# ittiam-systems/libxaac

Hardware: AMD Instinct MI355X
Metric: decoded audio frames/s (1024-spl IMDCT + complex QMF + HQ SBR + parametric stereo, HE-AACv2) (higher is better)
Workload: dtype int32

## Files before the change

### libxaac_amd/csrc/sbr_core.h

```cpp
#ifndef XAAC_SBR_CORE_H
#define XAAC_SBR_CORE_H

#include "fx.h"
#include "../../include/xaac_sbr.h"

#ifndef XS_TABLES_DECLARED
#define XS_TABLES_DECLARED
#if defined(__HIPCC__)
#define XAAC_TAB_QUAL static __device__ const
#include "tables_sbr.inc"
#undef XAAC_TAB_QUAL
#else
#include "tables_sbr.inc"
#endif
#endif

#define XS_MAXF XAAC_SBR_MAX_FREQ_COEFFS

FX_HD int32_t xs_shl(int32_t v, int s) { return (int32_t)((uint32_t)v << (s & 31)); }
FX_HD int32_t xs_sar(int32_t v, int s) { return v >> (s & 31); }
FX_HD int xs_pnorm32(int32_t a) { return fx_norm32(a); }
FX_HD int16_t xs_mult16_shl_sat(int16_t a, int16_t b) { return fx_sat16(((int32_t)a * b) >> 15); }
FX_HD int16_t xs_mult16_shl(int16_t a, int16_t b) { return (int16_t)(((int32_t)a * b) >> 15); }
FX_HD int16_t xs_mult16(int16_t a, int16_t b) { return (int16_t)(((int32_t)a * b) >> 16); }
// ... 317 lines not shown
  return r;
}

template <int HQ_, int NB_ = 64, int LD_ = 0, int NS_ = 32>
struct XsQmfT {
  static constexpr int HQ = HQ_;
  static constexpr int NB = NB_;
  static constexpr int LD = LD_;
  static constexpr int NS = NS_;
  static constexpr int OV = LD_ ? 0 : 6;
  static constexpr int IM = NB_;
  static constexpr int ROW = HQ_ ? 2 * NB_ : NB_;
  int32_t *p;
  FX_MEMBER int32_t &operator()(int slot, int band) const { return p[(slot + 2) * ROW + band]; }
  FX_MEMBER int32_t &im(int slot, int band) const { return p[(slot + 2) * ROW + IM + band]; }
};
typedef XsQmfT<0> XsQmf;
typedef XsQmfT<1> XsQmfHq;

struct XsCov {
  int32_t phi_11, phi_22, phi_01, phi_02, phi_12, d;
};

struct XsWork {
  int32_t bw_array[XAAC_SBR_MAX_PATCHES];
  union {
    int32_t fold_a[XS_MAXF + 8][2];
    int16_t nrg_est[2 * XS_MAXF];
  };
  int32_t fold_b[XS_MAXF + 8][4];
// ... 2132 lines not shown
      a0r = (int16_t)(xs_shl(fx_mul32x16(fx_sub_sat(0, tr), inv), norm + 1) >> 15);
    if (fx_abs_sat(ti) >= p11)
      reset = 1;
    else
      a0i = (int16_t)(xs_shl(fx_mul32x16(fx_sub_sat(0, ti), inv), norm + 1) >> 15);
  }
  if (fx_add_sat((int32_t)a0r * a0r, (int32_t)a0i * a0i) >= 0x40000000) reset = 1;
  if (fx_add_sat((int32_t)a1r * a1r, (int32_t)a1i * a1i) >= 0x40000000) reset = 1;
  if (reset) a0r = a0i = a1r = a1i = 0;
  a[0] = a0r;
  a[1] = a0i;
  a[2] = a1r;
  a[3] = a1i;
}

template <class Q>
FX_HD void xs_patch_band_hq(const xaac_sbr_header *h, const Q &x, int lb, int hb, const int16_t *alpha,
                            const int32_t *bw_array, int start_idx, int stop_idx) {
  constexpr int kBwCap = XAAC_SBR_MAX_PATCHES - 1 < XAAC_SBR_MAX_NOISE_VALUES ? XAAC_SBR_MAX_PATCHES - 1 : XAAC_SBR_MAX_NOISE_VALUES;
  int bord[kBwCap];
  XS_UNROLL
  for (int i = 0; i < kBwCap; i++) bord[i] = h->bw_borders[i];
  int bi = 0;
  bool on = true;
  XS_UNROLL
  for (int i = 0; i < kBwCap; i++) {
    on = on && hb >= bord[i];
    bi += on ? 1 : 0;
  }
  int16_t bw = (int16_t)(bw_array[bi] >> 16);
  const int16_t a0r = xs_mult16_shl_sat(bw, alpha[0]), a0i = xs_mult16_shl_sat(bw, alpha[1]);
  bw = xs_mult16_shl_sat(bw, bw);
  const int16_t a1r = xs_mult16_shl_sat(bw, alpha[2]), a1i = xs_mult16_shl_sat(bw, alpha[3]);
  const int n = stop_idx - start_idx;
  const bool filt = bw > 0;
  const int16_t c0r = filt ? a0r : (int16_t)0, c0i = filt ? a0i : (int16_t)0, c1r = filt ? a1r : (int16_t)0,
                c1i = filt ? a1i : (int16_t)0;
  int32_t p2r = x(start_idx - 2, lb), p2i = x.im(start_idx - 2, lb);
  int32_t p1r = x(start_idx - 1, lb), p1i = x.im(start_idx - 1, lb);
  XS_UNROLL4
  for (int i = 0; i < n; i++) {
    const int32_t cr = x(start_idx + i, lb), ci = x.im(start_idx + i, lb);
    int32_t acc = fx_sub(fx_add(fx_sub(fx_mul32x16(p1r, c0r), fx_mul32x16(p1i, c0i)), fx_mul32x16(p2r, c1r)),
                         fx_mul32x16(p2i, c1i));
    x(start_idx + i, hb) = fx_add(cr >> 2, fx_shlw(acc, 1));
    acc = fx_add(fx_add_sat(fx_add_sat(fx_mul32x16(p1r, c0i), fx_mul32x16(p1i, c0r)), fx_mul32x16(p2r, c1i)),
                 fx_mul32x16(p2i, c1r));
    x.im(start_idx + i, hb) = fx_add(ci >> 2, fx_shlw(acc, 1));
    p2r = p1r;
    p2i = p1i;
    p1r = cr;
    p1i = ci;
  }
}

template <class ST, class Q>
FX_HD void xs_hf_generator_hq(const XsCx &cx, const xaac_sbr_header *h, ST *st, const Q &x, XsWork *w,
                              int start_idx, int last_slot_offset, int max_qmf_subband, const int32_t *invf_mode,
                              const int32_t *invf_mode_prev) {
  const int num_patches = cx.uni(h->num_patches);
  const int stop_idx = cx.uni(h->num_columns) + last_slot_offset;
  XS_PAR(i, 0, XAAC_SBR_MAX_PATCHES) w->bw_array[i] = 0;
  cx.sync();
  xs_invfilt_level_emphasis(cx, st->bw_array_prev, h->num_if_bands, invf_mode, invf_mode_prev, w->bw_array);
  const int actual_stop = cx.uni(
      (int16_t)(h->patch[num_patches - 1].dst_start_band + h->patch[num_patches - 1].num_bands_in_patch));
  {
    const int nz = actual_stop < Q::NB ? Q::NB - actual_stop : 0;
    XS_PAR(c, 0, 2 * nz) {
      const int col = c < nz ? actual_stop + c : Q::IM + actual_stop + (c - nz);
      XS_UNROLL4
      for (int l = start_idx; l < stop_idx; l++) x(l, col) = 0;
    }
  }
  const int start_patch = cx.uni(h->start_patch), stop_patch = cx.uni(h->stop_patch);
  XS_PAR(k, start_patch, stop_patch) {
    x(-2, k) = st->lpc_real[0][k];
    x(-1, k) = st->lpc_real[1][k];
    x.im(-2, k) = st->lpc_imag[0][k];
    x.im(-1, k) = st->lpc_imag[1][k];
  }
  cx.sync();
  XS_T(12);
  XsLv al01, al23, src;
  al01.fill(0);
  al23.fill(0);
  const int ncov = Q::LD ? cx.uni(h->num_columns) : Q::NS + 6;
// ... 50 lines not shown
  XS_LANES(hb, 0, 64) wide |= src.own(hb) >= 0 && (hb < max_qmf_subband || hb >= max_qmf_subband + 32);
  if (cx.wave_or(wide) == 0 && max_qmf_subband >= 0 && stop_idx - start_idx >= 8) {
    XsLv idx;
    idx.fill(0);
    XS_LANES(l, 0, 64) idx.own(l) = (max_qmf_subband + (l & 31)) & 63;
    const XsLv src2 = src.gather(idx);
    XsLv srcc;
    srcc.fill(0);
    XS_LANES(l, 0, 64) srcc.own(l) = (max_qmf_subband + (l & 31) < 64) ? src2.own(l) : -1;
    const XsLv b01 = al01.gather(srcc), b23 = al23.gather(srcc);
    const int mid = start_idx + ((stop_idx - start_idx + 1) >> 1);
    XS_LANES(l, 0, 64) {
      const int lb = srcc.own(l), hb = max_qmf_subband + (l & 31);
      if (lb >= 0) {
        const int16_t alpha[4] = {xs_m(b01.own(l)), xs_e(b01.own(l)), xs_m(b23.own(l)), xs_e(b23.own(l))};
        xs_patch_band_hq(h, x, lb, hb, alpha, w->bw_array, l < 32 ? start_idx : mid, l < 32 ? mid : stop_idx);
      }
    }
  } else {
    const XsLv a01 = al01.gather(src), a23 = al23.gather(src);
    XS_LANES(hb, 0, 64) {
      const int lb = src.own(hb);
      if (lb >= 0) {
        const int16_t alpha[4] = {xs_m(a01.own(hb)), xs_e(a01.own(hb)), xs_m(a23.own(hb)), xs_e(a23.own(hb))};
        xs_patch_band_hq(h, x, lb, hb, alpha, w->bw_array, start_idx, stop_idx);
      }
    }
  }
  cx.sync();
  XS_T(14);
  XS_PAR(i, 0, h->num_if_bands) st->bw_array_prev[i] = w->bw_array[i];
  cx.sync();
}

struct XsPendingAdjust {
  int b0, b1, first_start, sh_ov, sh_main;
};
template <class ST, class Q>
FX_HD int xs_calc_sbrenvelope(const XsCx &cx, const xaac_sbr_header *h, const xaac_sbr_frame *f,
                              const int16_t *env_sf_all, const int16_t *noise_floor_all, ST *st, const Q &x,
// ... 425 lines not shown
FX_HD int xs_sbr_core_tail(const XsCx &cx, const xaac_sbr_header *h, const xaac_sbr_frame *f, const int16_t *env_sf_all,
                           const int16_t *noise_floor_all, ST *st, const Q &x, XsWork *w, const int16_t *rand_hi,
                           const XsBfp &b, XsPendingAdjust *pend = nullptr, const int32_t *sf_words = nullptr) {
  const int save_lb_scale = b.save_lb_scale, max_samp_val = b.max_samp_val;
  (void)max_samp_val;
  if (cx.uni(f->apply_processing)) {
    XsLv deg64;
    deg64.fill(0);
    const int n_env = cx.uni(f->num_env), nts = cx.uni(h->num_time_slots), ts = cx.uni(h->time_step);
    const int16_t last = fx_sat16((int32_t)cx.uni(f->border_vec[n_env]) - nts);
    if constexpr (!Q::HQ)
      xs_low_pow_hf_generator(cx, h, st, x, w, deg64, cx.uni(f->border_vec[0]) * ts, ts * last,
                              cx.uni(f->max_qmf_subband_aac), f->sbr_invf_mode, st->prev_invf_mode, max_samp_val);
    else
      xs_hf_generator_hq(cx, h, st, x, w, cx.uni(f->border_vec[0]) * ts, ts * last, cx.uni(f->max_qmf_subband_aac),
                         f->sbr_invf_mode, st->prev_invf_mode);
    XS_T(2);
    XS_ONE st->hb_scale = (int16_t)((st->ov_lb_scale < st->lb_scale ? st->ov_lb_scale : st->lb_scale) - 2);
    cx.sync();
    if (xs_calc_sbrenvelope(cx, h, f, env_sf_all, noise_floor_all, st, x, w, rand_hi, deg64, pend, sf_words)) return -1;
    XS_PAR(i, 0, h->num_if_bands) st->prev_invf_mode[i] = f->sbr_invf_mode[i];
    XS_ONE {
      st->prev_coupling_mode = f->coupling_mode;
      st->prev_max_qmf_subband_aac = f->max_qmf_subband_aac;
      st->prev_end_position = f->border_vec[f->num_env];
      st->prev_amp_res = f->amp_res;
    }
  } else {
    XS_ONE st->hb_scale = (int16_t)save_lb_scale;
  }
  cx.sync();
// ... 30 lines not shown
```

### libxaac_amd/csrc/sbr_core_kernel.h

```cpp
#ifndef XAAC_SBR_CORE_KERNEL_H
#define XAAC_SBR_CORE_KERNEL_H

#include <hip/hip_runtime_api.h>
#include <stdint.h>

#include "../../include/xaac_amd.h"

#define XAAC_SBR_X_ROWS 40
#define XAAC_SBR_X_WORDS (XAAC_SBR_X_ROWS * 64)
#define XAAC_SBR_NARROW_BANDS 48
#ifndef XAAC_SBR_CORE_HQ_WAVES
#define XAAC_SBR_CORE_HQ_WAVES 4
#endif

typedef struct XaacSbrCoreParams {
  int32_t n_ch;
  const xaac_sbr_header *header;
  const xaac_sbr_frame *frame;
  xaac_sbr_state *state;
  int32_t *x;
  int16_t *syn_par;
  int32_t *status;
  int32_t *defer_list, *defer_count;
  int32_t *work_counter;
  int32_t num_cu;
  int32_t counters_zeroed;
  int32_t qmf_slots;
  int32_t narrow_only;
} XaacSbrCoreParams;

#ifdef __cplusplus
extern "C" {
#endif
hipError_t xaac_launch_sbr_core_lp(const XaacSbrCoreParams *p, hipStream_t stream);
hipError_t xaac_launch_sbr_screen(const XaacSbrCoreParams *p, hipStream_t stream);
hipError_t xaac_launch_sbr_core_hq(const XaacSbrCoreParams *p, hipStream_t stream);
#ifdef __cplusplus
}
#endif
#endif
```

### libxaac_amd/csrc/sbr_core_kernel.hip

```cpp
#include <hip/hip_runtime.h>
#include <stddef.h>
#include <stdint.h>
#include <stdlib.h>

#ifdef XS_PROFILE
__shared__ long long xs_prof_last[4];
__shared__ unsigned xs_prof_acc[4][32];
#define XS_T(i)                                                  \
  do {                                                           \
    if ((threadIdx.x & 63) == 0) {                               \
      long long t_ = clock64();                                  \
      xs_prof_acc[threadIdx.x >> 6][i] += (unsigned)(t_ - xs_prof_last[threadIdx.x >> 6]); \
      xs_prof_last[threadIdx.x >> 6] = t_;                       \
    }                                                            \
  } while (0)
#endif
__shared__ int16_t xs_lds_inv_table[256];
__shared__ int16_t xs_lds_sqrt_table[258];
__shared__ int32_t xs_lds_rand_ph[568];
__shared__ int16_t xs_lds_rand_hi[568];
__shared__ int16_t xs_lds_small16[8 + 4 + 50];
__shared__ int32_t xs_lds_new_bw[16];
#define XS_TAB_LIMG(i) xs_lds_small16[i]
#define XS_TAB_SMOOTH(i) xs_lds_small16[8 + (i)]
// ... 341 lines not shown
  for (int j = 0; j < NR; j++)
    if (tid + THREADS * j < 568) {
      if (HQ)
        xs_lds_rand_ph[tid + THREADS * j] = tr[j];
      else
        xs_lds_rand_hi[tid + THREADS * j] = (int16_t)(tr[j] >> 16);
    }
#pragma unroll
  for (int j = 0; j < NI; j++)
    if (tid + THREADS * j < 256) xs_lds_inv_table[tid + THREADS * j] = ti[j];
#pragma unroll
  for (int j = 0; j < NS; j++)
    if (tid + THREADS * j < 257) xs_lds_sqrt_table[tid + THREADS * j] = ts[j];
}

}

#ifndef XS_LP_MIN_WAVES
#define XS_LP_MIN_WAVES 3
#endif
template <int HQ, int NB, int WAVES, int NS = 32>
__global__ __launch_bounds__(64 * WAVES, HQ ? 1 : XS_LP_MIN_WAVES) void xaac_sbr_core_kernel(XaacSbrCoreParams p) {
  __shared__ XsLds<HQ, NB> s[WAVES];
  const int lane = threadIdx.x & 63, wave = __builtin_amdgcn_readfirstlane(threadIdx.x >> 6);
  stage_tables<HQ, 64 * WAVES>(threadIdx.x);
  __syncthreads();
  if (XS_STAGGER_G > 1 && p.work_counter && p.n_ch >= 3 * (int)gridDim.x * WAVES) {
    const int g = ((int)blockIdx.x * WAVES + wave) % XS_STAGGER_G;
    for (int t = 0; t < g; t++) __builtin_amdgcn_s_sleep(XS_STAGGER_SLEEP);
  }
// ... 18 lines not shown
}

template <int HQ, int NS = 32>
__global__ __launch_bounds__(64) void xaac_sbr_core_list_kernel(XaacSbrCoreParams p) {
  __shared__ XsLds<HQ, 64> s;
  const int lane = threadIdx.x;
  const int n = *p.defer_count;
  if ((int)blockIdx.x >= n) return;
  stage_tables<HQ, 64>(lane);
  for (int j = blockIdx.x; j < n; j += gridDim.x) {
    xs_wave_sync();
    core_one<HQ, 64, NS>(p, p.defer_list[j], s, lane);
  }
}

template <int NS>
static hipError_t launch_sbr_core_lp(const XaacSbrCoreParams *p, hipStream_t stream) {
  XaacSbrCoreParams q = *p;
  q.work_counter = nullptr;
#ifndef XS_LP_WAVES
#define XS_LP_WAVES 2
#endif
  constexpr int W = XS_LP_WAVES;
#ifndef XS_LP_PERSISTENT
#define XS_LP_PERSISTENT 1
#endif
  if (XS_LP_PERSISTENT && p->work_counter && p->counters_zeroed) {
#ifndef XS_LP_WG_PER_CU
#define XS_LP_WG_PER_CU 5
#endif
// ... 31 lines not shown
    q.work_counter = nullptr;
    hipLaunchKernelGGL((xaac_sbr_core_kernel<1, 64, 1, NS>), dim3(p->n_ch), dim3(64), 0, stream, q);
    return hipGetLastError();
  }
  if (!p->counters_zeroed) {
    hipError_t e = hipMemsetAsync(p->defer_count, 0, 2 * sizeof(int32_t), stream);
    if (e != hipSuccess) return e;
  }
  constexpr int W = XAAC_SBR_CORE_HQ_WAVES;
  static int per_cu = 0;
  if (!per_cu) {
    const char *e = getenv("XAAC_CORE_WG_PER_CU");
    per_cu = e && atoi(e) > 0 ? atoi(e) : 2;
  }
  const int resident = per_cu * (p->num_cu > 0 ? p->num_cu : 256), need = (p->n_ch + W - 1) / W;
  hipLaunchKernelGGL((xaac_sbr_core_kernel<1, XAAC_SBR_NARROW_BANDS, W, NS>), dim3(need < resident ? need : resident), dim3(64 * W), 0,
                     stream, *p);
  if (p->narrow_only) return hipGetLastError();
  const int grid = p->n_ch < 64 ? p->n_ch : 64;
  hipLaunchKernelGGL((xaac_sbr_core_list_kernel<1, NS>), dim3(grid), dim3(64), 0, stream, *p);
  return hipGetLastError();
}

extern "C" hipError_t xaac_launch_sbr_core_hq(const XaacSbrCoreParams *p, hipStream_t stream) {
  return p->qmf_slots == 30 ? launch_sbr_core_hq<30>(p, stream) : launch_sbr_core_hq<32>(p, stream);
}

extern "C" hipError_t xaac_warm_sbr_core(void) {
  hipFuncAttributes a;
  return hipFuncGetAttributes(&a, reinterpret_cast<const void *>(&xaac_sbr_core_kernel<1, XAAC_SBR_NARROW_BANDS, XAAC_SBR_CORE_HQ_WAVES, 32>));
}
```

### libxaac_amd/csrc/sbr_qmf_kernel.h

```cpp
#ifndef XAAC_SBR_QMF_KERNEL_H
#define XAAC_SBR_QMF_KERNEL_H

#include <hip/hip_runtime_api.h>
#include <stdint.h>

#include "../../include/xaac_amd.h"
#include "../../include/xaac_sbr.h"

#ifndef XAAC_QMF_WAVES
#define XAAC_QMF_WAVES 1
#endif
#define XAAC_QMF_BLOCK (64 * XAAC_QMF_WAVES)
#define XAAC_QMF_ANA_LDS_PER_WAVE (2 * 1312 * 2 + 32 + 64 * 65 * 4)
#define XAAC_QMF_SYN_LDS_PER_WAVE_LP 21376
#define XAAC_QMF_SYN_LDS_PER_WAVE_HQ (64 * 129 * 4)

typedef struct XaacQmfAnaParams {
  int32_t n_ch, ch_fac, low_pow, usb, slot_stride;
  int32_t state_stride;
  int32_t qmf_ch_stride;
  const int16_t *pcm;
  xaac_qmf_ana_state *state;
  int32_t *qmf;
  const xaac_sbr_frame *frame;
  int32_t *zero_words;
  int32_t n_slots;
  const int16_t *refused;
} XaacQmfAnaParams;

typedef struct XaacQmfSynParams {
  int32_t n_ch, ch_fac, low_pow, lsb, usb, split, slot_stride;
  int32_t state_stride, qmf_ch_stride;
  int32_t scale_stride;
  int32_t per_ch_bands;
  int32_t down_sample;
  const int32_t *qmf;
  const int16_t *scale;
  xaac_qmf_syn_state *state;
  int16_t *pcm;
  int32_t pcm_ch_stride, pcm_sample_stride;
// ... 43 lines not shown
```

### libxaac_amd/csrc/sbr_qmf_kernel.hip

```cpp
#include <hip/hip_runtime.h>
#include <stdint.h>

#include "sbr_qmf.h"
#include "sbr_qmf_kernel.h"

namespace {

constexpr int kHist = 288 + 1024;

__device__ __forceinline__ int ana_ring_pos(int wr, int a) {
  int p = wr + 32 + a;
  return p >= 320 ? p - 320 : p;
}

template <int NS = 32>
__device__ __forceinline__ int ana_phase_after_frame(int phase) {
  int f1 = phase, f2 = phase + 64;
  for (int s = 0; s < NS; s++) {
    f1 += 64;
    f2 += 64;
    int t = f1;
    f1 = f2;
    f2 = t;
    if (f2 > 640) {
// ... 13 lines not shown
}

template <bool LP, int NS = 32>
__global__ __launch_bounds__(XAAC_QMF_BLOCK) void xaac_qmf_analysis_kernel(XaacQmfAnaParams p) {
  extern __shared__ __attribute__((aligned(16))) char smem[];
  const int lane = threadIdx.x & 63;
  const int wave = __builtin_amdgcn_readfirstlane(threadIdx.x >> 6);
  char *wbase = smem + wave * XAAC_QMF_ANA_LDS_PER_WAVE;
  int16_t *hist = reinterpret_cast<int16_t *>(wbase);
  int32_t *z = reinterpret_cast<int32_t *>(wbase + 2 * kHist * 2 + 32);

  int32_t coef[5];
#pragma unroll
  for (int j = 0; j < 5; j++) coef[j] = xaac_qmf_qmf_c[2 * lane + 128 * j];

  if (p.zero_words && blockIdx.x == 0 && threadIdx.x < 2) p.zero_words[threadIdx.x] = 0;
  const int n_pairs = (p.n_ch + 1) >> 1;
  const int waves_total = gridDim.x * XAAC_QMF_WAVES;
  for (int pair = blockIdx.x * XAAC_QMF_WAVES + wave; pair < n_pairs; pair += waves_total) {
    int wr_v[2] = {0, 0}, ph_v[2] = {0, 0};
    {
      constexpr int NP = 32 * NS / 64;
      int16_t hr[2][5], hp[2][NP];
#pragma unroll
      for (int c = 0; c < 2; c++) {
        const int ch = 2 * pair + c;
        if (ch < p.n_ch) {
          const xaac_qmf_ana_state *st = reinterpret_cast<const xaac_qmf_ana_state *>(
              reinterpret_cast<const char *>(p.state) + (size_t)ch * p.state_stride);
          wr_v[c] = st->wr;
          ph_v[c] = st->phase;
// ... 102 lines not shown
        st->phase = (int16_t)ph_new;
      }
    }
  }
}

template <int NS = 32>
__global__ __launch_bounds__(128) void xaac_qmf_analysis_hq_kernel(XaacQmfAnaParams p) {
  __shared__ int16_t hist[2][kHist];
  __shared__ int32_t tile[2 * 64 * 33];
  const int lane = threadIdx.x & 63;
  const int w = __builtin_amdgcn_readfirstlane(threadIdx.x >> 6);
  const int pair = blockIdx.x;
  const int chw = 2 * pair + w;
  const bool live = chw < p.n_ch;
  if (p.zero_words && blockIdx.x == 0 && threadIdx.x < 2) p.zero_words[threadIdx.x] = 0;
  xaac_qmf_ana_state *st = reinterpret_cast<xaac_qmf_ana_state *>(reinterpret_cast<char *>(p.state) + (size_t)(live ? chw : 0) * p.state_stride);
  int wr = 0, phase_old = 0;
  int rot_apply = 0, rot_sub = 0, rot_usb = 0;
  const bool rot_live = p.frame && 2 * pair + (lane >> 5) < p.n_ch;
  if (rot_live) {
    const int ch = 2 * pair + (lane >> 5);
    const xaac_sbr_frame *f = p.frame + ch;
    const xaac_sbr_state *sst = reinterpret_cast<const xaac_sbr_state *>(reinterpret_cast<const char *>(p.state) + (size_t)ch * p.state_stride);
    rot_apply = f->apply_processing;
    rot_sub = f->max_qmf_subband_aac;
    rot_usb = sst->codec_usb;
  }
  {
    int16_t *h = hist[w];
    if (live) {
// ... 830 lines not shown
```

### libxaac_amd/csrc/xaac_abi.cpp

```cpp
#include <hip/hip_runtime_api.h>
#include "build_id.h"

#include <cstdint>
#include <cstdlib>
#include <new>

#include "../../include/xaac_amd.h"
#include "imdct_kernel.h"
#include "sbr_qmf_kernel.h"
#include "sbr_core_kernel.h"
#include "sbr_ld_core_kernel.h"
#include "sbr_ps_kernel.h"
#include "limiter_kernel.h"
#include "esbr_qmf_kernel.h"
#include "usac_imdct_kernel.h"
#include "imdct960_kernel.h"
#include "imdct_ld_kernel.h"
#include "esbr_core_kernel.h"
#include "hbe_kernel.h"
#include "pvc_kernel.h"
#include "aac_tools_kernel.h"
#include <cmath>
#include <cstddef>
#include <cstring>
// ... 628 lines not shown
  if (b->n_ch % b->in_ch_fac || b->n_ch % b->out_ch_fac) return XAAC_FATAL_BAD_ARG;
  if (b->n_ch == 0) return XAAC_OK;
  if (!b->pcm_in || !b->header || !b->frame || !b->state || !b->pcm_out || !b->workspace) return XAAC_FATAL_NULL_ARG;
  if (b->workspace_bytes < xaac_sbr_lp_workspace_bytes(b->n_ch)) return XAAC_FATAL_BAD_ARG;
  if (!hip_ok(hipSetDevice(c->device))) return XAAC_FATAL_HIP;
  int32_t *x = reinterpret_cast<int32_t *>(((uintptr_t)b->workspace + 255) & ~(uintptr_t)255);
  int16_t *par = reinterpret_cast<int16_t *>(x + (size_t)b->n_ch * XAAC_SBR_X_WORDS);
  char *st = reinterpret_cast<char *>(b->state);
  XaacQmfAnaParams pa = {};
  pa.n_ch = b->n_ch; pa.ch_fac = b->in_ch_fac; pa.low_pow = 1; pa.usb = 32; pa.slot_stride = 64; pa.n_slots = ns;
  pa.state_stride = (int32_t)sizeof(xaac_sbr_state); pa.qmf_ch_stride = XAAC_SBR_X_WORDS;
  pa.pcm = b->pcm_in;
  pa.state = reinterpret_cast<xaac_qmf_ana_state *>(st + offsetof(xaac_sbr_state, ana_ring));
  pa.qmf = x + (2 + 6) * 64;
  int32_t *counters = reinterpret_cast<int32_t *>(((uintptr_t)(par + (size_t)b->n_ch * 8) + 63) & ~(uintptr_t)63);
  pa.zero_words = counters;
  if (ns == 30) {
    XaacSbrCoreParams sc = {};
    sc.n_ch = b->n_ch; sc.header = b->header; sc.frame = b->frame; sc.state = b->state; sc.syn_par = par; sc.qmf_slots = ns;
    if (!hip_ok(xaac_launch_sbr_screen(&sc, c->stream))) return XAAC_FATAL_HIP;
    pa.refused = par;
  }
  if (!hip_ok(xaac_launch_qmf_analysis(&pa, qmf_grid(c, b->n_ch, 0), c->stream))) return XAAC_FATAL_HIP;
  XaacSbrCoreParams pc = {};
  pc.n_ch = b->n_ch; pc.header = b->header; pc.frame = b->frame; pc.state = b->state; pc.x = x; pc.syn_par = par;
  pc.status = b->status;
  pc.defer_count = counters; pc.work_counter = counters + 1; pc.num_cu = c->num_cu; pc.counters_zeroed = 1;
  pc.qmf_slots = ns;
  if (!hip_ok(xaac_launch_sbr_core_lp(&pc, c->stream))) return XAAC_FATAL_HIP;
  XaacQmfSynParams ps = {};
  ps.n_ch = b->n_ch; ps.ch_fac = b->out_ch_fac; ps.low_pow = 1; ps.lsb = 0; ps.usb = 0; ps.split = 6; ps.n_slots = ns;
// ... 2 lines not shown
  ps.scale_stride = 8; ps.per_ch_bands = 1;
  ps.qmf = x + 2 * 64; ps.scale = par; ps.dbg = XAAC_DBG_BUF(b->status, b->n_ch);
  ps.state = reinterpret_cast<xaac_qmf_syn_state *>(st + offsetof(xaac_sbr_state, syn_ring));
  ps.pcm = b->pcm_out;
  const int grid = qmf_grid(c, b->n_ch, 2);
  if (!hip_ok(xaac_launch_qmf_synthesis(&ps, grid, c->stream))) return XAAC_FATAL_HIP;
  c->last_grid = grid; c->last_block = XAAC_QMF_BLOCK; c->last_lds = XAAC_QMF_WAVES * XAAC_QMF_SYN_LDS_PER_WAVE_LP;
  return XAAC_OK;
}

int32_t xaac_sbr_lp_process_batch(xaac_ctx *c, const xaac_sbr_lp_batch *b) { return sbr_lp_run(c, b, 32); }
int32_t xaac_sbr_lp960_process_batch(xaac_ctx *c, const xaac_sbr_lp_batch *b) { return sbr_lp_run(c, b, 30); }

uint64_t xaac_sbr_hq_workspace_bytes(int32_t n_ch, int32_t with_ps) {
  if (n_ch < 0) return 0;
  uint64_t per = 2 * XAAC_SBR_X_WORDS * 4 + 8 * 2 + 4;
  if (with_ps) per += 32 * 128 * 4 + 8 * 2;
  return (uint64_t)n_ch * per + 512 + 128;
}

uint64_t xaac_sbr_eld_workspace_bytes(int32_t n_ch) {
  return n_ch > 0 ? (uint64_t)n_ch * (16 * 128 * 4 + 8 * 2) + 512 : 0;
}
int32_t xaac_sbr_eld_process_batch(xaac_ctx *c, const xaac_sbr_eld_batch *b) {
  if (!c || !b) return XAAC_FATAL_NULL_ARG;
  if (b->n_ch < 0 || (b->n_slots != 16 && b->n_slots != 15)) return XAAC_FATAL_BAD_ARG;
  if ((b->in_ch_fac != 1 && b->in_ch_fac != 2) || (b->out_ch_fac != 1 && b->out_ch_fac != 2)) return XAAC_FATAL_BAD_ARG;
  if (b->n_ch % b->in_ch_fac || b->n_ch % b->out_ch_fac) return XAAC_FATAL_BAD_ARG;
  if (b->n_ch == 0) return XAAC_OK;
  if (!b->pcm_in || !b->header || !b->frame || !b->state || !b->pcm_out || !b->workspace) return XAAC_FATAL_NULL_ARG;
  if (b->workspace_bytes < xaac_sbr_eld_workspace_bytes(b->n_ch)) return XAAC_FATAL_BAD_ARG;
  if (!hip_ok(hipSetDevice(c->device))) return XAAC_FATAL_HIP;
  const size_t n = (size_t)b->n_ch;
// ... 38 lines not shown
  const size_t n = (size_t)b->n_ch;
  const int xw = 2 * XAAC_SBR_X_WORDS;
  int32_t *x = reinterpret_cast<int32_t *>(((uintptr_t)b->workspace + 255) & ~(uintptr_t)255);
  int32_t *xr = x + n * xw;
  int16_t *par_l = reinterpret_cast<int16_t *>(xr + (with_ps ? n * 32 * 128 : 0));
  int16_t *par_r = par_l + n * 8;
  char *st = reinterpret_cast<char *>(b->state);
  XaacQmfAnaParams pa = {};
  pa.n_ch = b->n_ch; pa.ch_fac = b->in_ch_fac; pa.low_pow = 0; pa.usb = 32; pa.slot_stride = 128; pa.n_slots = ns;
  pa.state_stride = (int32_t)sizeof(xaac_sbr_state); pa.qmf_ch_stride = xw;
  pa.pcm = b->pcm_in;
  pa.state = reinterpret_cast<xaac_qmf_ana_state *>(st + offsetof(xaac_sbr_state, ana_ring));
  pa.qmf = x + (2 + 6) * 128;
  pa.frame = b->frame;
  int32_t *counters = reinterpret_cast<int32_t *>(((uintptr_t)(par_l + n * 8 * (with_ps ? 2 : 1)) + 63) & ~(uintptr_t)63);
  pa.zero_words = counters;
  if (ns == 30) {
    XaacSbrCoreParams sc = {};
    sc.n_ch = b->n_ch; sc.header = b->header; sc.frame = b->frame; sc.state = b->state; sc.syn_par = par_l; sc.qmf_slots = ns;
    if (!hip_ok(xaac_launch_sbr_screen(&sc, c->stream))) return XAAC_FATAL_HIP;
    pa.refused = par_l;
  }
  if (!hip_ok(xaac_launch_qmf_analysis(&pa, qmf_grid(c, b->n_ch, 1), c->stream))) return XAAC_FATAL_HIP;
  XaacSbrCoreParams pc = {};
  pc.n_ch = b->n_ch; pc.header = b->header; pc.frame = b->frame; pc.state = b->state; pc.x = x; pc.syn_par = par_l;
  pc.status = b->status;
  pc.defer_count = counters; pc.work_counter = counters + 1; pc.defer_list = counters + 2; pc.num_cu = c->num_cu;
  pc.counters_zeroed = 1;
  pc.narrow_only = b->max_band_hint == XAAC_SBR_NARROW_BANDS ? 1 : 0;
  pc.qmf_slots = ns;
  if (!hip_ok(xaac_launch_sbr_core_hq(&pc, c->stream))) return XAAC_FATAL_HIP;
  if (with_ps) {
    XaacPsParams pp = {};
    pp.n_slots = ns;
    pp.n = b->n_ch; pp.x = x; pp.xr = xr; pp.header = b->header; pp.sbr_frame = b->frame; pp.frame = b->ps_frame;
    pp.state = b->ps_state; pp.sbr_state = b->state; pp.par_l = par_l; pp.par_r = par_r; pp.status = b->status; pp.dbg = XAAC_DBG_BUF(b->status, b->n_ch);
    if (!hip_ok(xaac_launch_ps(&pp, c->stream))) return XAAC_FATAL_HIP;
  }
  if (with_ps) {
    XaacQmfSynPairParams pq = {};
    pq.n = b->n_ch; pq.split = 6; pq.n_slots = ns;
    pq.qmf[0] = x + 2 * 128; pq.qmf_stride[0] = xw; pq.scale[0] = par_l;
// ... 82 lines not shown
```

Before: 16.35 million.

## Split HQ SBR core into separate HF-generation and envelope-adjust kernels

Replaces the single fused HQ SBR core kernel with two kernels for 32-slot frames. The first runs the HF generator on a narrow LDS window of low bands, and the second runs envelope adjustment on a high-band window, with a per-channel handover word passing state between them. The smaller per-kernel LDS footprint is meant to allow more waves resident per CU. The cost is an extra global round trip of the QMF buffer, a third kernel launch, and extra counters in a larger workspace. Channels that do not fit the narrow windows fall back to the deferred list kernel.

```diff
diff --git a/libxaac_amd/csrc/sbr_core.h b/libxaac_amd/csrc/sbr_core.h
--- a/libxaac_amd/csrc/sbr_core.h
+++ b/libxaac_amd/csrc/sbr_core.h
@@ -355,6 +355,9 @@
   int32_t *p;
   FX_MEMBER int32_t &operator()(int slot, int band) const { return p[(slot + 2) * ROW + band]; }
   FX_MEMBER int32_t &im(int slot, int band) const { return p[(slot + 2) * ROW + IM + band]; }
+  static FX_MEMBER XsQmfT window(int32_t *block, int band0, int first_slot) {
+    return XsQmfT{block - ((first_slot + 2) * ROW + band0)};
+  }
 };
 typedef XsQmfT<0> XsQmf;
 typedef XsQmfT<1> XsQmfHq;
@@ -2517,8 +2520,8 @@
   a[3] = a1i;
 }
 
-template <class Q>
-FX_HD void xs_patch_band_hq(const xaac_sbr_header *h, const Q &x, int lb, int hb, const int16_t *alpha,
+template <class Q, class QD>
+FX_HD void xs_patch_band_hq(const xaac_sbr_header *h, const Q &x, const QD &xd, int lb, int hb, const int16_t *alpha,
                             const int32_t *bw_array, int start_idx, int stop_idx) {
   constexpr int kBwCap = XAAC_SBR_MAX_PATCHES - 1 < XAAC_SBR_MAX_NOISE_VALUES ? XAAC_SBR_MAX_PATCHES - 1 : XAAC_SBR_MAX_NOISE_VALUES;
   int bord[kBwCap];
@@ -2546,10 +2549,10 @@
     const int32_t cr = x(start_idx + i, lb), ci = x.im(start_idx + i, lb);
     int32_t acc = fx_sub(fx_add(fx_sub(fx_mul32x16(p1r, c0r), fx_mul32x16(p1i, c0i)), fx_mul32x16(p2r, c1r)),
                          fx_mul32x16(p2i, c1i));
-    x(start_idx + i, hb) = fx_add(cr >> 2, fx_shlw(acc, 1));
+    xd(start_idx + i, hb) = fx_add(cr >> 2, fx_shlw(acc, 1));
     acc = fx_add(fx_add_sat(fx_add_sat(fx_mul32x16(p1r, c0i), fx_mul32x16(p1i, c0r)), fx_mul32x16(p2r, c1i)),
                  fx_mul32x16(p2i, c1r));
-    x.im(start_idx + i, hb) = fx_add(ci >> 2, fx_shlw(acc, 1));
+    xd.im(start_idx + i, hb) = fx_add(ci >> 2, fx_shlw(acc, 1));
     p2r = p1r;
     p2i = p1i;
     p1r = cr;
@@ -2557,10 +2560,10 @@
   }
 }
 
-template <class ST, class Q>
-FX_HD void xs_hf_generator_hq(const XsCx &cx, const xaac_sbr_header *h, ST *st, const Q &x, XsWork *w,
+template <class ST, class Q, class W, class QD>
+FX_HD void xs_hf_generator_hq(const XsCx &cx, const xaac_sbr_header *h, ST *st, const Q &x, W *w,
                               int start_idx, int last_slot_offset, int max_qmf_subband, const int32_t *invf_mode,
-                              const int32_t *invf_mode_prev) {
+                              const int32_t *invf_mode_prev, const QD &xd) {
   const int num_patches = cx.uni(h->num_patches);
   const int stop_idx = cx.uni(h->num_columns) + last_slot_offset;
   XS_PAR(i, 0, XAAC_SBR_MAX_PATCHES) w->bw_array[i] = 0;
@@ -2569,11 +2572,11 @@
   const int actual_stop = cx.uni(
       (int16_t)(h->patch[num_patches - 1].dst_start_band + h->patch[num_patches - 1].num_bands_in_patch));
   {
-    const int nz = actual_stop < Q::NB ? Q::NB - actual_stop : 0;
+    const int nz = actual_stop < QD::NB ? QD::NB - actual_stop : 0;
     XS_PAR(c, 0, 2 * nz) {
-      const int col = c < nz ? actual_stop + c : Q::IM + actual_stop + (c - nz);
+      const int col = c < nz ? actual_stop + c : QD::IM + actual_stop + (c - nz);
       XS_UNROLL4
-      for (int l = start_idx; l < stop_idx; l++) x(l, col) = 0;
+      for (int l = start_idx; l < stop_idx; l++) xd(l, col) = 0;
     }
   }
   const int start_patch = cx.uni(h->start_patch), stop_patch = cx.uni(h->stop_patch);
@@ -2654,7 +2657,7 @@
       const int lb = srcc.own(l), hb = max_qmf_subband + (l & 31);
       if (lb >= 0) {
         const int16_t alpha[4] = {xs_m(b01.own(l)), xs_e(b01.own(l)), xs_m(b23.own(l)), xs_e(b23.own(l))};
-        xs_patch_band_hq(h, x, lb, hb, alpha, w->bw_array, l < 32 ? start_idx : mid, l < 32 ? mid : stop_idx);
+        xs_patch_band_hq(h, x, xd, lb, hb, alpha, w->bw_array, l < 32 ? start_idx : mid, l < 32 ? mid : stop_idx);
       }
     }
   } else {
@@ -2663,7 +2666,7 @@
       const int lb = src.own(hb);
       if (lb >= 0) {
         const int16_t alpha[4] = {xs_m(a01.own(hb)), xs_e(a01.own(hb)), xs_m(a23.own(hb)), xs_e(a23.own(hb))};
-        xs_patch_band_hq(h, x, lb, hb, alpha, w->bw_array, start_idx, stop_idx);
+        xs_patch_band_hq(h, x, xd, lb, hb, alpha, w->bw_array, start_idx, stop_idx);
       }
     }
   }
@@ -3119,7 +3122,7 @@
                               cx.uni(f->max_qmf_subband_aac), f->sbr_invf_mode, st->prev_invf_mode, max_samp_val);
     else
       xs_hf_generator_hq(cx, h, st, x, w, cx.uni(f->border_vec[0]) * ts, ts * last, cx.uni(f->max_qmf_subband_aac),
-                         f->sbr_invf_mode, st->prev_invf_mode);
+                         f->sbr_invf_mode, st->prev_invf_mode, x);
     XS_T(2);
     XS_ONE st->hb_scale = (int16_t)((st->ov_lb_scale < st->lb_scale ? st->ov_lb_scale : st->lb_scale) - 2);
     cx.sync();
diff --git a/libxaac_amd/csrc/sbr_core_kernel.h b/libxaac_amd/csrc/sbr_core_kernel.h
--- a/libxaac_amd/csrc/sbr_core_kernel.h
+++ b/libxaac_amd/csrc/sbr_core_kernel.h
@@ -9,6 +9,11 @@
 #define XAAC_SBR_X_ROWS 40
 #define XAAC_SBR_X_WORDS (XAAC_SBR_X_ROWS * 64)
 #define XAAC_SBR_NARROW_BANDS 48
+#define XAAC_SBR_SPLIT_LOW_BANDS 24
+#define XAAC_SBR_SPLIT_HIGH_BANDS 28
+#ifndef XAAC_SBR_CORE_SPLIT
+#define XAAC_SBR_CORE_SPLIT 1
+#endif
 #ifndef XAAC_SBR_CORE_HQ_WAVES
 #define XAAC_SBR_CORE_HQ_WAVES 4
 #endif
@@ -27,6 +32,7 @@
   int32_t counters_zeroed;
   int32_t qmf_slots;
   int32_t narrow_only;
+  int32_t *adj_counter, *handover;
 } XaacSbrCoreParams;
 
 #ifdef __cplusplus
diff --git a/libxaac_amd/csrc/sbr_core_kernel.hip b/libxaac_amd/csrc/sbr_core_kernel.hip
--- a/libxaac_amd/csrc/sbr_core_kernel.hip
+++ b/libxaac_amd/csrc/sbr_core_kernel.hip
@@ -379,6 +379,358 @@
     if (tid + THREADS * j < 257) xs_lds_sqrt_table[tid + THREADS * j] = ts[j];
 }
 
+
+constexpr int kSplitLow = XAAC_SBR_SPLIT_LOW_BANDS, kSplitHigh = XAAC_SBR_SPLIT_HIGH_BANDS;
+static_assert(kSplitLow <= 32 && kSplitHigh <= 32, "a window's real | imaginary columns fit the wave side by side");
+#ifdef XS_PROFILE
+constexpr bool kSplitOn = false;
+#else
+constexpr bool kSplitOn = XAAC_SBR_CORE_SPLIT != 0;
+#endif
+constexpr int32_t kNotSplit = -1;
+
+struct XsWorkBw {
+  int32_t bw_array[XAAC_SBR_MAX_PATCHES];
+};
+template <int NL>
+struct XsLdsHf {
+  int32_t x[XAAC_SBR_X_ROWS * 2 * NL];
+  XsLdsState st;
+  xaac_sbr_header h;
+  int32_t f_head[kFrameHeadBytes / 4];
+  XsWorkBw w;
+};
+template <int NHI>
+struct XsLdsAdj {
+  int32_t x[(XAAC_SBR_X_ROWS - 2) * 2 * NHI];
+  XsLdsState st;
+  xaac_sbr_header h;
+  int32_t f_head[kFrameHeadBytes / 4];
+  int32_t noise_floor[sizeof(((xaac_sbr_frame *)0)->int_noise_floor) / 4];
+  XsWork w;
+};
+
+template <int NL, int NHI>
+__device__ __forceinline__ int hf_one(const XaacSbrCoreParams &p, const int ch, XsLdsHf<NL> &s, const int lane) {
+  constexpr int NS = 32, ROWG = 128, XWG = 2 * XAAC_SBR_X_WORDS;
+  typedef XsQmfT<1, NL, 0, NS> Q;
+  typedef XsQmfT<1, 64, 0, NS> QG;
+  constexpr int ROW = Q::ROW;
+  xaac_sbr_state *gst = p.state + ch;
+  int32_t *gx = p.x + (size_t)ch * XWG;
+  const int32_t *gstw = reinterpret_cast<const int32_t *>(gst);
+  constexpr int NH = (sizeof(xaac_sbr_header) / 4 + 63) / 64, NT = (kTailWords + 63) / 64, NOV = 6 * ROWG / 64, NAS = NS;
+  int32_t r_h[NH], r_f, r_hd = 0, r_t[NT], r_ov[NOV], r_an[NAS];
+  {
+    const int32_t *gh = reinterpret_cast<const int32_t *>(p.header + ch), *gf = reinterpret_cast<const int32_t *>(p.frame + ch);
+#pragma unroll
+    for (int j = 0; j < NH; j++) r_h[j] = lane + 64 * j < (int)(sizeof(xaac_sbr_header) / 4) ? gh[lane + 64 * j] : 0;
+    r_f = lane < kFrameHeadBytes / 4 ? gf[lane] : 0;
+    if (lane < 2) r_hd = gstw[kHeadOff / 4 + lane];
+#pragma unroll
+    for (int j = 0; j < NT; j++) r_t[j] = lane + 64 * j < kTailWords ? gstw[kTailOff / 4 + lane + 64 * j] : 0;
+    const int32_t *gov = gstw + offsetof(xaac_sbr_state, overlap) / 4;
+#pragma unroll
+    for (int j = 0; j < NOV; j++) r_ov[j] = gov[lane + 64 * j];
+#pragma unroll
+    for (int j = 0; j < NAS; j++) r_an[j] = gx[(8 + j) * ROWG + (lane & 31) + ((lane & 32) ? 64 : 0)];
+  }
+  const xaac_sbr_frame *f = reinterpret_cast<const xaac_sbr_frame *>(s.f_head);
+  {
+#pragma unroll
+    for (int j = 0; j < NH; j++)
+      if (lane + 64 * j < (int)(sizeof(xaac_sbr_header) / 4)) reinterpret_cast<int32_t *>(&s.h)[lane + 64 * j] = r_h[j];
+    if (lane < kFrameHeadBytes / 4) s.f_head[lane] = r_f;
+    int32_t *m = reinterpret_cast<int32_t *>(&s.st);
+    if (lane < 2) m[lane] = r_hd;
+#pragma unroll
+    for (int j = 0; j < NT; j++)
+      if (lane + 64 * j < kTailWords) m[2 + lane + 64 * j] = r_t[j];
+    for (int i = lane; i < 2 * ROW; i += 64) s.x[i] = 0;
+  }
+  int32_t above = 0;
+#pragma unroll
+  for (int j = 0; j < NOV; j++) above |= lane < XAAC_SBR_NARROW_BANDS ? 0 : r_ov[j];
+  xs_wave_sync();
+
+  const XsCx cx = {lane, 64};
+  const Q x = {s.x};
+  const QG xg = {gx};
+  if (lane == 0) s.st.lb_scale = 0;
+  const int refused = xs_side_info_bad(cx, &s.h, f, &s.st, 0, NS);
+  const int apply = __builtin_amdgcn_readfirstlane((int)f->apply_processing);
+  const int old_lsb = __builtin_amdgcn_readfirstlane((int)s.st.prev_max_qmf_subband_aac);
+  const int new_lsb = __builtin_amdgcn_readfirstlane((int)f->max_qmf_subband_aac);
+  {
+    int32_t top = 0, src_top = 0;
+    if (!refused) {
+      const int32_t lim[4] = {s.st.syn_usb, s.st.syn_lsb, s.st.codec_usb, s.st.prev_max_qmf_subband_aac};
+      for (int i = 0; i < 4; i++) top = lim[i] > top ? lim[i] : top;
+      if (apply) {
+        top = s.h.sub_band_end > top ? s.h.sub_band_end : top;
+        top = f->max_qmf_subband_aac > top ? f->max_qmf_subband_aac : top;
+        if (lane <= s.h.num_sf_bands[1] && s.h.freq_band_tbl_hi[lane] > top) top = s.h.freq_band_tbl_hi[lane];
+        if (lane <= s.h.num_sf_bands[0] && s.h.freq_band_tbl_lo[lane] > top) top = s.h.freq_band_tbl_lo[lane];
+        if (lane < s.h.num_patches) {
+          const xaac_sbr_patch *pp = &s.h.patch[lane];
+          const int a = pp->src_end_band + pp->dst_end_band, b = pp->dst_start_band + pp->num_bands_in_patch;
+          top = a > top ? a : top;
+          top = b > top ? b : top;
+          src_top = pp->src_end_band;
+        }
+      }
+    }
+    if (cx.wave_max(top) > XAAC_SBR_NARROW_BANDS || cx.wave_or(above) != 0) return 2;
+    const int sb_start = __builtin_amdgcn_readfirstlane((int)s.h.sub_band_start), sb_end = __builtin_amdgcn_readfirstlane((int)s.h.sub_band_end);
+    const int n_pat = __builtin_amdgcn_readfirstlane((int)s.h.num_patches), stop_patch = __builtin_amdgcn_readfirstlane((int)s.h.stop_patch);
+    const bool fits = !refused && apply && !(new_lsb != old_lsb && old_lsb > 0) && new_lsb <= NL && stop_patch <= new_lsb &&
+                      cx.wave_max(src_top) <= new_lsb && n_pat >= 1 && sb_end - sb_start <= NHI && sb_end >= new_lsb;
+    if (!fits) return 1;
+  }
+  xs_rescale_x_overlap(cx, &s.h, f, &s.st, x);
+  xs_wave_sync();
+  if (lane == 0) {
+    s.st.st_lb_scale = 0;
+    s.st.lb_scale = -8;
+  }
+  xs_wave_sync();
+  const int usb = __builtin_amdgcn_readfirstlane((int)s.st.codec_usb);
+  int32_t m_ov = 1, m_an = 1;
+  const bool low_ov = lane < usb, low_an = (lane & 31) < usb;
+#pragma unroll
+  for (int j = 0; j < NOV; j++) m_ov |= low_ov ? fx_abs_nrm(r_ov[j]) : 0;
+#pragma unroll
+  for (int j = 0; j < NAS; j++) m_an |= low_an ? fx_abs_nrm(r_an[j]) : 0;
+  const int reserve = xs_pnorm32(cx.wave_or(m_an)), reserve_ov1 = xs_pnorm32(cx.wave_or(m_ov));
+  const XsBfp b = xs_bfp_shifts<1>(cx, &s.st, usb, reserve, reserve_ov1);
+  if (b.sh_ov != 0) {
+#pragma unroll
+    for (int j = 0; j < NOV; j++) r_ov[j] = low_ov ? xs_adjust_word(r_ov[j], b.sh_ov) : r_ov[j];
+  }
+  if (b.sh_main != 0) {
+#pragma unroll
+    for (int j = 0; j < NAS; j++) r_an[j] = low_an ? xs_adjust_word(r_an[j], b.sh_main) : r_an[j];
+  }
+  if (lane < NL) {
+#pragma unroll
+    for (int j = 0; j < NOV; j++) s.x[(2 + (j >> 1)) * ROW + (j & 1) * NL + lane] = r_ov[j];
+  }
+  if ((lane & 31) < NL) {
+#pragma unroll
+    for (int j = 0; j < NAS; j++) s.x[(8 + j) * ROW + (lane & 31) + ((lane & 32) ? Q::IM : 0)] = r_an[j];
+  }
+  if (lane >= usb) {
+#pragma unroll
+    for (int j = 0; j < NOV; j++) gx[2 * ROWG + 64 * j + lane] = r_ov[j];
+  }
+#pragma unroll
+  for (int j = 0; j < NAS; j++) gx[(8 + j) * ROWG + 32 + (lane & 31) + ((lane & 32) ? 64 : 0)] = 0;
+  xs_wave_sync();
+  __builtin_amdgcn_s_waitcnt(0x0F70);
+  {
+    const int n_env = cx.uni(f->num_env), nts = cx.uni(s.h.num_time_slots), ts = cx.uni(s.h.time_step);
+    const int16_t last = fx_sat16((int32_t)cx.uni(f->border_vec[n_env]) - nts);
+    xs_hf_generator_hq(cx, &s.h, &s.st, x, &s.w, cx.uni(f->border_vec[0]) * ts, ts * last, new_lsb, f->sbr_invf_mode,
+                       s.st.prev_invf_mode, xg);
+    if (lane == 0) s.st.hb_scale = (int16_t)((s.st.ov_lb_scale < s.st.lb_scale ? s.st.ov_lb_scale : s.st.lb_scale) - 2);
+  }
+  xs_wave_sync();
+  {
+    constexpr int NW = (NS + 6) * 2;
+    const bool mine = lane < usb;
+    const int lane_l = mine ? lane : 0;
+#pragma unroll
+    for (int j0 = 0; j0 < NW; j0 += 8) {
+      int32_t t[8];
+#pragma unroll
+      for (int j = 0; j < 8; j++)
+        if (j0 + j < NW) t[j] = s.x[(2 + ((j0 + j) >> 1)) * ROW + ((j0 + j) & 1) * NL + lane_l];
+      if (mine) {
+#pragma unroll
+        for (int j = 0; j < 8; j++)
+          if (j0 + j < NW) gx[2 * ROWG + 64 * (j0 + j) + lane] = t[j];
+      }
+    }
+    int32_t *gw = reinterpret_cast<int32_t *>(gst);
+    if (mine) {
+#pragma unroll
+      for (int j = 0; j < 6; j++) gw[offsetof(xaac_sbr_state, overlap) / 4 + 64 * j + lane] = s.x[(2 + NS + (j >> 1)) * ROW + (j & 1) * NL + lane_l];
+    }
+    const int32_t *m = reinterpret_cast<const int32_t *>(&s.st);
+    if (lane < 2) gw[kHeadOff / 4 + lane] = m[lane];
+    copy_words(gw + kTailOff / 4, m + 2, kTailWords, lane);
+    if (lane == 0) p.handover[ch] = (int32_t)(((uint32_t)s.h.sub_band_start << 16) | (uint16_t)b.save_lb_scale);
+  }
+  return 0;
+}
+
+template <int NHI>
+__device__ __forceinline__ void adj_one(const XaacSbrCoreParams &p, const int ch, XsLdsAdj<NHI> &s, const int lane) {
+  constexpr int NS = 32, ROWG = 128, XWG = 2 * XAAC_SBR_X_WORDS, NR = NS + 6;
+  typedef XsQmfT<1, NHI, 0, NS> Q;
+  constexpr int ROW = Q::ROW;
+  int32_t rec = lane == 0 ? p.handover[ch] : 0;
+  rec = __builtin_amdgcn_readfirstlane(rec);
+  if (rec == kNotSplit) return;
+  const int c0 = rec >> 16, save_lb_scale = (int16_t)rec;
+  xaac_sbr_state *gst = p.state + ch;
+  int32_t *gx = p.x + (size_t)ch * XWG;
+  const int32_t *gstw = reinterpret_cast<const int32_t *>(gst);
+  constexpr int NH = (sizeof(xaac_sbr_header) / 4 + 63) / 64, NT = (kTailWords + 63) / 64;
+  constexpr int NNF = sizeof(s.noise_floor) / 4;
+  constexpr int NSF = (sizeof(((xaac_sbr_frame *)0)->int_env_sf_arr) / 4 + 63) / 64;
+  const int col = lane & 31;
+  const bool held = col < NHI && c0 + col < 64;
+  const int gcol = ((lane & 32) ? 64 : 0) + (held ? c0 + col : 0), lcol = ((lane & 32) ? Q::IM : 0) + (held ? col : 0);
+  int32_t r_h[NH], r_f, r_nf = 0, r_hd = 0, r_t[NT], r_sf[NSF];
+  {
+    const int32_t *gh = reinterpret_cast<const int32_t *>(p.header + ch), *gf = reinterpret_cast<const int32_t *>(p.frame + ch);
+#pragma unroll
+    for (int j = 0; j < NH; j++) r_h[j] = lane + 64 * j < (int)(sizeof(xaac_sbr_header) / 4) ? gh[lane + 64 * j] : 0;
+    r_f = lane < kFrameHeadBytes / 4 ? gf[lane] : 0;
+    if (lane < NNF) r_nf = reinterpret_cast<const int32_t *>(p.frame[ch].int_noise_floor)[lane];
+#pragma unroll
+    for (int j = 0; j < NSF; j++)
+      r_sf[j] = lane + 64 * j < (int)(sizeof(((xaac_sbr_frame *)0)->int_env_sf_arr) / 4) ? reinterpret_cast<const int32_t *>(p.frame[ch].int_env_sf_arr)[lane + 64 * j] : 0;
+    if (lane < 2) r_hd = gstw[kHeadOff / 4 + lane];
+#pragma unroll
+    for (int j = 0; j < NT; j++) r_t[j] = lane + 64 * j < kTailWords ? gstw[kTailOff / 4 + lane + 64 * j] : 0;
+  }
+#pragma unroll
+  for (int r0 = 0; r0 < NR; r0 += NR / 2) {
+    int32_t t[NR / 2];
+#pragma unroll
+    for (int j = 0; j < NR / 2; j++) t[j] = gx[(2 + r0 + j) * ROWG + gcol];
+    if (held) {
+#pragma unroll
+      for (int j = 0; j < NR / 2; j++) s.x[(r0 + j) * ROW + lcol] = t[j];
+    }
+  }
+  const xaac_sbr_frame *f = reinterpret_cast<const xaac_sbr_frame *>(s.f_head);
+  {
+#pragma unroll
+    for (int j = 0; j < NH; j++)
+      if (lane + 64 * j < (int)(sizeof(xaac_sbr_header) / 4)) reinterpret_cast<int32_t *>(&s.h)[lane + 64 * j] = r_h[j];
+    if (lane < kFrameHeadBytes / 4) s.f_head[lane] = r_f;
+    if (lane < NNF) s.noise_floor[lane] = r_nf;
+    int32_t *m = reinterpret_cast<int32_t *>(&s.st);
+    if (lane < 2) m[lane] = r_hd;
+#pragma unroll
+    for (int j = 0; j < NT; j++)
+      if (lane + 64 * j < kTailWords) m[2 + lane + 64 * j] = r_t[j];
+  }
+  xs_wave_sync();
+  const XsCx cx = {lane, 64};
+  const Q x = Q::window(s.x, c0, 0);
+  XsPendingAdjust pend = {0, 0, 0, 0, 0};
+  int rc = 0;
+  {
+    XsLv deg64;
+    deg64.fill(0);
+    if (xs_calc_sbrenvelope(cx, &s.h, f, p.frame[ch].int_env_sf_arr, reinterpret_cast<const int16_t *>(s.noise_floor), &s.st, x, &s.w,
+                            (const int16_t *)nullptr, deg64, &pend, r_sf)) {
+      rc = -1;
+    } else {
+      XS_PAR(i, 0, s.h.num_if_bands) s.st.prev_invf_mode[i] = f->sbr_invf_mode[i];
+      if (lane == 0) {
+        s.st.prev_coupling_mode = f->coupling_mode;
+        s.st.prev_max_qmf_subband_aac = f->max_qmf_subband_aac;
+        s.st.prev_end_position = f->border_vec[f->num_env];
+        s.st.prev_amp_res = f->amp_res;
+      }
+    }
+  }
+  xs_wave_sync();
+  int lane_o = lane;
+  XS_KEEP(lane_o);
+  const int col_o = lane_o & 31;
+  const bool held_o = col_o < NHI && c0 + col_o < 64;
+  const int gcol_o = ((lane_o & 32) ? 64 : 0) + (held_o ? c0 + col_o : 0), lcol_o = ((lane_o & 32) ? Q::IM : 0) + (held_o ? col_o : 0);
+  const int usb = __builtin_amdgcn_readfirstlane((int)s.st.codec_usb);
+  int32_t *gw = reinterpret_cast<int32_t *>(gst);
+  int32_t ovn[6];
+#pragma unroll
+  for (int j = 0; j < 6; j++) ovn[j] = gx[(2 + NS + (j >> 1)) * ROWG + 64 * (j & 1) + lane_o];
+  int32_t lpc[4];
+  if (rc == 0) {
+#pragma unroll
+    for (int j = 0; j < 4; j++) lpc[j] = gx[(2 + NS - 2 + (j & 1)) * ROWG + 64 * (j >> 1) + col_o];
+  }
+  if (lane_o == 0) {
+    int16_t *par = p.syn_par + 8 * (size_t)ch;
+    par[0] = s.st.lb_scale;
+    par[1] = s.st.ov_lb_scale;
+    par[2] = s.st.hb_scale;
+    par[3] = s.st.st_syn_scale;
+    par[4] = s.st.syn_lsb;
+    par[5] = s.st.syn_usb;
+    par[6] = 0;
+    par[7] = 0;
+    s.st.ov_lb_scale = (int16_t)save_lb_scale;
+    if (p.status) p.status[ch] = rc;
+  }
+  xs_wave_sync();
+  {
+    const int band = c0 + col_o;
+    const bool adj_band = held_o && band >= pend.b0 && band < pend.b1;
+    const auto counts = [](int sh, int &l, int &r) {
+      sh = sh > 31 ? 31 : (sh < -31 ? -31 : sh);
+      l = sh > 0 ? sh : 0;
+      r = sh < 0 ? -sh : 0;
+    };
+    int ov_l, ov_r, mn_l, mn_r;
+    counts(pend.sh_ov, ov_l, ov_r);
+    counts(pend.sh_main, mn_l, mn_r);
+    const bool wr = held_o && band >= usb;
+#pragma unroll
+    for (int j0 = 0; j0 < NR; j0 += 8) {
+      int32_t t[8];
+#pragma unroll
+      for (int j = 0; j < 8; j++)
+        if (j0 + j < NR) {
+          const int row = j0 + j;
+          int32_t v = s.x[row * ROW + lcol_o];
+          if (row < NS) {
+            const int sl = row < pend.first_start ? ov_l : mn_l, sr = row < pend.first_start ? ov_r : mn_r;
+            const int32_t w = (int32_t)((uint32_t)v << sl) >> sr;
+            v = adj_band ? w : v;
+          }
+          t[j] = v;
+        }
+      if (wr) {
+#pragma unroll
+        for (int j = 0; j < 8; j++)
+          if (j0 + j < NR) gx[(2 + j0 + j) * ROWG + gcol_o] = t[j];
+      }
+    }
+#pragma unroll
+    for (int j = 0; j < 6; j++) {
+      const int row = j >> 1, b64 = lane_o;
+      const bool in_win = b64 >= c0 && b64 < c0 + NHI;
+      int32_t v = s.x[(NS + row) * ROW + (j & 1) * Q::IM + (in_win ? b64 - c0 : 0)];
+      v = in_win ? v : ovn[j];
+      if (NS + row < pend.first_start && b64 >= pend.b0 && b64 < pend.b1) {
+        const int sh = pend.sh_ov > 31 ? 31 : (pend.sh_ov < -31 ? -31 : pend.sh_ov);
+        v = sh > 0 ? (int32_t)((uint32_t)v << sh) : (v >> -sh);
+      }
+      if (b64 >= usb) gw[offsetof(xaac_sbr_state, overlap) / 4 + 64 * j + lane_o] = v;
+    }
+    int32_t *m = reinterpret_cast<int32_t *>(&s.st);
+    if (rc == 0 && col_o < usb) {
+      const int k = col_o;
+      if (lane_o < 32) {
+        m[2 + k] = lpc[0];
+        m[2 + 32 + k] = lpc[1];
+        m[2 + 64 + k] = lpc[2];
+        m[2 + 96 + k] = lpc[3];
+      }
+    }
+    xs_wave_sync();
+    if (lane_o < 2) gw[kHeadOff / 4 + lane_o] = m[lane_o];
+    copy_words(gw + kTailOff / 4, m + 2, kTailWords, lane_o);
+  }
+}
+
 }
 
 #ifndef XS_LP_MIN_WAVES
@@ -427,6 +779,55 @@
   }
 }
 
+
+template <int WAVES>
+__global__ __launch_bounds__(64 * WAVES, 3) void xaac_sbr_core_hf_kernel(XaacSbrCoreParams p) {
+  __shared__ XsLdsHf<kSplitLow> s[WAVES];
+  const int lane = threadIdx.x & 63, wave = __builtin_amdgcn_readfirstlane(threadIdx.x >> 6);
+  stage_tables<1, 64 * WAVES>(threadIdx.x);
+  __syncthreads();
+  if (XS_STAGGER_G > 1 && p.n_ch >= 3 * (int)gridDim.x * WAVES) {
+    const int g = ((int)blockIdx.x * WAVES + wave) % XS_STAGGER_G;
+    for (int t = 0; t < g; t++) __builtin_amdgcn_s_sleep(XS_STAGGER_SLEEP);
+  }
+  for (;;) {
+    int ch = 0;
+    if (lane == 0) ch = atomicAdd(p.work_counter, 1);
+    ch = __builtin_amdgcn_readfirstlane(ch);
+    if (ch >= p.n_ch) break;
+    const int r = hf_one<kSplitLow, kSplitHigh>(p, ch, s[wave], lane);
+    if (r != 0 && lane == 0) {
+      p.handover[ch] = kNotSplit;
+      if (r == 2 && p.narrow_only) {
+        if (p.status) p.status[ch] = XAAC_FATAL_BAD_ARG;
+      } else {
+        p.defer_list[atomicAdd(p.defer_count, 1)] = ch;
+      }
+    }
+    xs_wave_sync();
+  }
+}
+
+template <int WAVES>
+__global__ __launch_bounds__(64 * WAVES, 3) void xaac_sbr_core_adj_kernel(XaacSbrCoreParams p) {
+  __shared__ XsLdsAdj<kSplitHigh> s[WAVES];
+  const int lane = threadIdx.x & 63, wave = __builtin_amdgcn_readfirstlane(threadIdx.x >> 6);
+  stage_tables<1, 64 * WAVES>(threadIdx.x);
+  __syncthreads();
+  if (XS_STAGGER_G > 1 && p.n_ch >= 3 * (int)gridDim.x * WAVES) {
+    const int g = ((int)blockIdx.x * WAVES + wave) % XS_STAGGER_G;
+    for (int t = 0; t < g; t++) __builtin_amdgcn_s_sleep(XS_STAGGER_SLEEP);
+  }
+  for (;;) {
+    int ch = 0;
+    if (lane == 0) ch = atomicAdd(p.adj_counter, 1);
+    ch = __builtin_amdgcn_readfirstlane(ch);
+    if (ch >= p.n_ch) break;
+    adj_one<kSplitHigh>(p, ch, s[wave], lane);
+    xs_wave_sync();
+  }
+}
+
 template <int NS>
 static hipError_t launch_sbr_core_lp(const XaacSbrCoreParams *p, hipStream_t stream) {
   XaacSbrCoreParams q = *p;
@@ -488,10 +889,17 @@
     per_cu = e && atoi(e) > 0 ? atoi(e) : 2;
   }
   const int resident = per_cu * (p->num_cu > 0 ? p->num_cu : 256), need = (p->n_ch + W - 1) / W;
+  const int grid = p->n_ch < 64 ? p->n_ch : 64;
+  if (kSplitOn && NS == 32 && p->adj_counter && p->handover && p->counters_zeroed) {
+    const int res3 = 3 * (p->num_cu > 0 ? p->num_cu : 256);
+    hipLaunchKernelGGL((xaac_sbr_core_hf_kernel<W>), dim3(need < res3 ? need : res3), dim3(64 * W), 0, stream, *p);
+    hipLaunchKernelGGL((xaac_sbr_core_adj_kernel<W>), dim3(need < res3 ? need : res3), dim3(64 * W), 0, stream, *p);
+    hipLaunchKernelGGL((xaac_sbr_core_list_kernel<1, NS>), dim3(grid), dim3(64), 0, stream, *p);
+    return hipGetLastError();
+  }
   hipLaunchKernelGGL((xaac_sbr_core_kernel<1, XAAC_SBR_NARROW_BANDS, W, NS>), dim3(need < resident ? need : resident), dim3(64 * W), 0,
                      stream, *p);
   if (p->narrow_only) return hipGetLastError();
-  const int grid = p->n_ch < 64 ? p->n_ch : 64;
   hipLaunchKernelGGL((xaac_sbr_core_list_kernel<1, NS>), dim3(grid), dim3(64), 0, stream, *p);
   return hipGetLastError();
 }
diff --git a/libxaac_amd/csrc/sbr_qmf_kernel.h b/libxaac_amd/csrc/sbr_qmf_kernel.h
--- a/libxaac_amd/csrc/sbr_qmf_kernel.h
+++ b/libxaac_amd/csrc/sbr_qmf_kernel.h
@@ -24,6 +24,7 @@
   int32_t *qmf;
   const xaac_sbr_frame *frame;
   int32_t *zero_words;
+  int32_t zero_count;
   int32_t n_slots;
   const int16_t *refused;
 } XaacQmfAnaParams;
diff --git a/libxaac_amd/csrc/sbr_qmf_kernel.hip b/libxaac_amd/csrc/sbr_qmf_kernel.hip
--- a/libxaac_amd/csrc/sbr_qmf_kernel.hip
+++ b/libxaac_amd/csrc/sbr_qmf_kernel.hip
@@ -51,7 +51,7 @@
 #pragma unroll
   for (int j = 0; j < 5; j++) coef[j] = xaac_qmf_qmf_c[2 * lane + 128 * j];
 
-  if (p.zero_words && blockIdx.x == 0 && threadIdx.x < 2) p.zero_words[threadIdx.x] = 0;
+  if (p.zero_words && blockIdx.x == 0 && (int)threadIdx.x < (p.zero_count > 2 ? p.zero_count : 2)) p.zero_words[threadIdx.x] = 0;
   const int n_pairs = (p.n_ch + 1) >> 1;
   const int waves_total = gridDim.x * XAAC_QMF_WAVES;
   for (int pair = blockIdx.x * XAAC_QMF_WAVES + wave; pair < n_pairs; pair += waves_total) {
@@ -184,7 +184,7 @@
   const int pair = blockIdx.x;
   const int chw = 2 * pair + w;
   const bool live = chw < p.n_ch;
-  if (p.zero_words && blockIdx.x == 0 && threadIdx.x < 2) p.zero_words[threadIdx.x] = 0;
+  if (p.zero_words && blockIdx.x == 0 && (int)threadIdx.x < (p.zero_count > 2 ? p.zero_count : 2)) p.zero_words[threadIdx.x] = 0;
   xaac_qmf_ana_state *st = reinterpret_cast<xaac_qmf_ana_state *>(reinterpret_cast<char *>(p.state) + (size_t)(live ? chw : 0) * p.state_stride);
   int wr = 0, phase_old = 0;
   int rot_apply = 0, rot_sub = 0, rot_usb = 0;
diff --git a/libxaac_amd/csrc/xaac_abi.cpp b/libxaac_amd/csrc/xaac_abi.cpp
--- a/libxaac_amd/csrc/xaac_abi.cpp
+++ b/libxaac_amd/csrc/xaac_abi.cpp
@@ -666,7 +666,7 @@
   pa.state = reinterpret_cast<xaac_qmf_ana_state *>(st + offsetof(xaac_sbr_state, ana_ring));
   pa.qmf = x + (2 + 6) * 64;
   int32_t *counters = reinterpret_cast<int32_t *>(((uintptr_t)(par + (size_t)b->n_ch * 8) + 63) & ~(uintptr_t)63);
-  pa.zero_words = counters;
+  pa.zero_words = counters; pa.zero_count = 4;
   if (ns == 30) {
     XaacSbrCoreParams sc = {};
     sc.n_ch = b->n_ch; sc.header = b->header; sc.frame = b->frame; sc.state = b->state; sc.syn_par = par; sc.qmf_slots = ns;
@@ -699,9 +699,9 @@
 
 uint64_t xaac_sbr_hq_workspace_bytes(int32_t n_ch, int32_t with_ps) {
   if (n_ch < 0) return 0;
-  uint64_t per = 2 * XAAC_SBR_X_WORDS * 4 + 8 * 2 + 4;
+  uint64_t per = 2 * XAAC_SBR_X_WORDS * 4 + 8 * 2 + 4 + 4;
   if (with_ps) per += 32 * 128 * 4 + 8 * 2;
-  return (uint64_t)n_ch * per + 512 + 128;
+  return (uint64_t)n_ch * per + 512 + 128 + 16;
 }
 
 uint64_t xaac_sbr_eld_workspace_bytes(int32_t n_ch) {
@@ -770,7 +770,7 @@
   pa.qmf = x + (2 + 6) * 128;
   pa.frame = b->frame;
   int32_t *counters = reinterpret_cast<int32_t *>(((uintptr_t)(par_l + n * 8 * (with_ps ? 2 : 1)) + 63) & ~(uintptr_t)63);
-  pa.zero_words = counters;
+  pa.zero_words = counters; pa.zero_count = 4;
   if (ns == 30) {
     XaacSbrCoreParams sc = {};
     sc.n_ch = b->n_ch; sc.header = b->header; sc.frame = b->frame; sc.state = b->state; sc.syn_par = par_l; sc.qmf_slots = ns;
@@ -781,7 +781,8 @@
   XaacSbrCoreParams pc = {};
   pc.n_ch = b->n_ch; pc.header = b->header; pc.frame = b->frame; pc.state = b->state; pc.x = x; pc.syn_par = par_l;
   pc.status = b->status;
-  pc.defer_count = counters; pc.work_counter = counters + 1; pc.defer_list = counters + 2; pc.num_cu = c->num_cu;
+  pc.defer_count = counters; pc.work_counter = counters + 1; pc.adj_counter = counters + 2; pc.defer_list = counters + 4;
+  pc.handover = counters + 4 + n; pc.num_cu = c->num_cu;
   pc.counters_zeroed = 1;
   pc.narrow_only = b->max_band_hint == XAAC_SBR_NARROW_BANDS ? 1 : 0;
   pc.qmf_slots = ns;
```

After: 13.71 million. -16.1%, worse.
